# PriUVBio/optiland_Pr

Hardware: AMD Instinct MI355X
Metric: ray-surface intersections/sec at 1M pupil rays, 10-surf double-Gauss (higher is better)
Workload: dtype f64

## Files before the change

### optiland_pr_amd/csrc/ort_fastpath.h

```cpp
#pragma once

#include "ort_core.h"

namespace ort {
namespace fast {

#ifdef ORT_NO_HOSTCONST
#define ORT_TWO_R(s) (2.0 * (s).radius)
#define ORT_ONE_PLUS_K(s) (1.0 + (s).conic)
#define ORT_R_SQ(s) ((s).radius * (s).radius)
#define ORT_U_SQ(u, u_sq) ((u) * (u))
#else
#define ORT_TWO_R(s) ((s).two_r)
#define ORT_ONE_PLUS_K(s) ((s).one_plus_k)
#define ORT_R_SQ(s) ((s).r_sq)
#define ORT_U_SQ(u, u_sq) (u_sq)
#endif

#ifdef ORT_FAST_NOCHECK
#define ORT_CHK(bad, cond) ((void)0)
#else
#define ORT_CHK(bad, cond) ((bad) = (bad) | (cond))
#endif

ORT_INLINE bool is_pos_zero(double v) {
#if defined(__HIP_DEVICE_COMPILE__)
  return __builtin_amdgcn_class(v, 1 << 6);
#else
  return v == 0.0 && !signbit(v);
#endif
}

ORT_INLINE double sqrt(double x, bool& bad) {
#if defined(__HIP_DEVICE_COMPILE__)
  const double y = __builtin_amdgcn_rsq(x);
  double g = x * y;
  double h = y * 0.5;
  const double r = fma(-h, g, 0.5);
  g = fma(g, r, g);
  h = fma(h, r, h);
  double d = fma(-g, g, x);
  g = fma(d, h, g);
  d = fma(-g, g, x);
  g = fma(d, h, g);
  ORT_CHK(bad, !(x >= 0x1p-767));
  return g;
#else
  (void)bad;
  return ::sqrt(x);
#endif
}

ORT_INLINE double sqrt_ge1(double x, bool& bad) {
#if defined(__HIP_DEVICE_COMPILE__)
  const double y = __builtin_amdgcn_rsq(x);
  double g = x * y;
  double h = y * 0.5;
  const double r = fma(-h, g, 0.5);
  g = fma(g, r, g);
  h = fma(h, r, h);
  double d = fma(-g, g, x);
  g = fma(d, h, g);
  d = fma(-g, g, x);
  g = fma(d, h, g);
  (void)bad;
  return g;
#else
  (void)bad;
  return ::sqrt(x);
#endif
}

ORT_INLINE SharedDiv shared_div(double b, bool& bad) {
  SharedDiv d;
  d.b = b;
  d.ok = true;
#if defined(__HIP_DEVICE_COMPILE__)
  double y = __builtin_amdgcn_rcp(b);
  double e = fma(-b, y, 1.0);
  y = fma(y, e, y);
  e = fma(-b, y, 1.0);
  y = fma(y, e, y);
  d.y = y;
  ORT_CHK(bad, !(::fabs(b) <= 0x1p300));
#else
  (void)bad;
  d.y = 0.0;
#endif
  return d;
}

ORT_INLINE SharedDiv shared_div_ge1(double b, bool& bad) {
  SharedDiv d;
  d.b = b;
  d.ok = true;
  (void)bad;
#if defined(__HIP_DEVICE_COMPILE__)
  double y = __builtin_amdgcn_rcp(b);
  double e = fma(-b, y, 1.0);
  y = fma(y, e, y);
  e = fma(-b, y, 1.0);
  y = fma(y, e, y);
  d.y = y;
#else
  (void)bad;
  d.y = 0.0;
#endif
  return d;
}

ORT_INLINE double quot(double a, const SharedDiv& d) {
#if defined(__HIP_DEVICE_COMPILE__)
  const double q0 = a * d.y;
  const double r = fma(-d.b, q0, a);
  return fma(r, d.y, q0);
#else
  return a / d.b;
#endif
}

ORT_INLINE double quot_pos(double a, const SharedDiv& d) {
#if defined(__HIP_DEVICE_COMPILE__)
  const double q0 = a * d.y;
  const double rn = fma(d.b, q0, -a);
  return fma(-rn, d.y, q0);
#else
  return a / d.b;
#endif
}

ORT_INLINE bool num_ok(double a) { return ::fabs(a) >= 0x1p-300; }

ORT_INLINE double sdiv(double a, const SharedDiv& d, bool& bad) {
  ORT_CHK(bad, !num_ok(a));
  return quot(a, d);
}
ORT_INLINE double sdiv0(double a, const SharedDiv& d, bool& bad) {
  ORT_CHK(bad, !(num_ok(a) || is_pos_zero(a)));
  return quot(a, d);
}

ORT_INLINE double div(double a, double b, bool& bad) {
  const SharedDiv d = shared_div(b, bad);
  return sdiv0(a, d, bad);
}

ORT_INLINE Ray generate_ray(const ort_segment& s, double px, double py,
                            const ort_apodization* apod, bool& bad) {
  Ray r;
  double x0, y0;
  if (s.mode == ORT_GEN_INFINITE) {
    x0 = px * s.epd / 2.0 * s.vx + s.x_off;
    y0 = py * s.epd / 2.0 * s.vy + s.y_off;
  } else {
    x0 = s.x_off;
    y0 = s.y_off;
  }
  const double z0 = s.z0;
  double x1, y1;
  if (s.mode == ORT_GEN_TELECENTRIC) {
    x1 = px * s.vx + x0;
    y1 = py * s.vy + y0;
  } else {
    x1 = px * s.epd * s.vx / 2.0;
    y1 = py * s.epd * s.vy / 2.0;
  }
  const double z1 = s.epl;
  const double dx = x1 - x0, dy = y1 - y0, dz = z1 - z0;
  const double mag = sqrt(dx * dx + dy * dy + dz * dz, bad);
  ORT_CHK(bad, (mag < 1e-9));
  const SharedDiv dm = shared_div(mag, bad);
  ORT_CHK(bad, !((num_ok(dx) || dx == 0.0) && (num_ok(dy) || dy == 0.0) &&
                 (num_ok(dz) || dz == 0.0)));
  r.L = quot_pos(dx, dm);
  r.M = quot_pos(dy, dm);
  r.N = quot_pos(dz, dm);
  r.x = x0;
  r.y = y0;
  r.z = z0;
  r.i = apod ? apodize(*apod, px, py) : 1.0;
  r.opd = 0.0;
  r.att = 0.0;
  return r;
}

ORT_INLINE bool state_ok(const Ray& r) {
  constexpr double kMax = 0x1p1000;
  return ::fabs(r.x) < kMax && ::fabs(r.y) < kMax && ::fabs(r.z) < kMax &&
         ::fabs(r.L) < kMax && ::fabs(r.M) < kMax && ::fabs(r.N) < kMax && ::fabs(r.opd) < kMax;
}

ORT_INLINE double distance_plane(const Ray& r, bool& bad) { return div(-r.z, r.N, bad); }

ORT_INLINE double distance_conic(const Ray& r, const ort_surface& s, bool radius_inf,
                                 bool& bad) {
  if (radius_inf) {
    const double Ns = ::fabs(r.N) > 1e-14 ? r.N : 1e-14;
    return div(-r.z, Ns, bad);
  }
  const double R = s.radius, k = s.conic;
  const double N2 = r.N * r.N;
  const double z2 = r.z * r.z;
  double a, b, c;
  if (k == 0.0) {
    a = r.L * r.L + r.M * r.M + N2;
    b = 2.0 * (r.L * r.x + r.M * r.y - r.N * R + r.N * r.z);
    c = 0.0 - ORT_TWO_R(s) * r.z + r.x * r.x + r.y * r.y + z2;
  } else {
    a = k * N2 + r.L * r.L + r.M * r.M + N2;
    b = 2.0 * (k * r.N * r.z + r.L * r.x + r.M * r.y - r.N * R + r.N * r.z);
    c = k * z2 - ORT_TWO_R(s) * r.z + r.x * r.x + r.y * r.y + z2;
  }
  const double d = b * b - 4.0 * a * c;
  const double sd = sqrt(d, bad);
  const SharedDiv a2 = shared_div(2.0 * a, bad);
  const double n1 = -b + sd, n2 = -b - sd;
  ORT_CHK(bad, !(num_ok(n1) && num_ok(n2)));
  const double t1 = quot_pos(n1, a2);
  const double t2 = quot_pos(n2, a2);
  const double z1 = r.z + t1 * r.N;
  const double zz2 = r.z + t2 * r.N;
  return ::fabs(z1) <= ::fabs(zz2) ? t1 : t2;
}

ORT_INLINE void normal_conic_rcp(double x, double y, const ort_surface& s, double& nx,
                                 double& ny, double& nz, bool& bad) {
  const double r2 = x * x + y * y;
  const double a = ORT_ONE_PLUS_K(s) * r2;
  const double q0 = a * s.inv_r2;
  const double q = fma(fma(-ORT_R_SQ(s), q0, a), s.inv_r2, q0);
  const double denom = s.radius * sqrt(1.0 - q, bad);
  const SharedDiv dd = shared_div(denom, bad);
  const double dfdx = sdiv0(x, dd, bad);
  const double dfdy = sdiv0(y, dd, bad);
  const double mag = sqrt_ge1(dfdx * dfdx + dfdy * dfdy + 1.0, bad);
  const SharedDiv dm = shared_div_ge1(mag, bad);
  nx = quot_pos(dfdx, dm);
  ny = quot_pos(dfdy, dm);
  nz = quot(-1.0, dm);
}

ORT_INLINE double align_normal(const Ray& r, double& nx, double& ny, double& nz, bool& bad) {
#ifdef ORT_NO_SIGN_XOR
  return ::ort::align_normal(r, nx, ny, nz);
#endif
  const double dot = r.L * nx + r.M * ny + r.N * nz;
  ORT_CHK(bad, !(::fabs(dot) > 0.0));
  const uint64_t sb = (uint64_t)__double_as_longlong(dot) & 0x8000000000000000ull;
  nx = __longlong_as_double((long long)((uint64_t)__double_as_longlong(nx) ^ sb));
  ny = __longlong_as_double((long long)((uint64_t)__double_as_longlong(ny) ^ sb));
  nz = __longlong_as_double((long long)((uint64_t)__double_as_longlong(nz) ^ sb));
  return ::fabs(dot);
}

ORT_INLINE void refract(Ray& r, double nx, double ny, double nz, double u, double u_sq,
                        bool& bad) {
  const double dot = align_normal(r, nx, ny, nz, bad);
  const double root = sqrt(1.0 - ORT_U_SQ(u, u_sq) * (1.0 - dot * dot), bad);
  const double L0 = r.L, M0 = r.M, N0 = r.N;
  r.L = u * L0 + nx * root - u * nx * dot;
  r.M = u * M0 + ny * root - u * ny * dot;
  r.N = u * N0 + nz * root - u * nz * dot;
}

ORT_INLINE void refract_flat(Ray& r, double u, double u_sq, bool& bad) {
  ORT_CHK(bad, !(::fabs(r.N) > 0.0));
  const double root = sqrt(1.0 - ORT_U_SQ(u, u_sq) * (1.0 - r.N * r.N), bad);
  const double uN = u * r.N;
  const double sroot = ::copysign(root, r.N);
  r.L = u * r.L + 0.0;
  r.M = u * r.M + 0.0;
  r.N = (uN + sroot) - uN;
}

ORT_INLINE double quot_signed(double a, const SharedDiv& d) {
  return d.b > 0.0 ? quot_pos(a, d) : quot(a, d);
}
ORT_INLINE bool num_ok0(double a) { return num_ok(a) || a == 0.0; }

ORT_INLINE SharedDiv shared_div_pos(double b) {
  bool unused = false;
  return shared_div_ge1(b, unused);
}
ORT_INLINE bool lens_range(double R) { return ::fabs(R) <= 0x1p149; }

ORT_INLINE void slope_out(double dfdx, double dfdy, double& nx, double& ny, double& nz,
                          bool& bad) {
#ifdef ORT_SLOPE_MAXCHK
  ORT_CHK(bad, !(::fabs(dfdx) < 7e13 && ::fabs(dfdy) < 7e13));
#else
  ORT_CHK(bad, !(dfdx * dfdx + dfdy * dfdy + 1.0 < 1e28));
#endif
  nx = dfdx;
  ny = dfdy;
  nz = -1.0;
}

ORT_INLINE void unit_normal_from_slope(double dfdx, double dfdy, double& nx, double& ny,
                                       double& nz, bool& bad) {
  const double mag = sqrt_ge1(dfdx * dfdx + dfdy * dfdy + 1.0, bad);
  const SharedDiv dm = shared_div_ge1(mag, bad);
  ORT_CHK(bad, !(num_ok0(dfdx) && num_ok0(dfdy)));
  nx = quot_pos(dfdx, dm);
  ny = quot_pos(dfdy, dm);
  nz = quot(-1.0, dm);
}

template <class PD>
ORT_INLINE double sagnorm_even(double x, double y, const ort_surface& s, PD C,
                               int nc, int mode, double& nx, double& ny, double& nz,
                               bool& bad) {
  const double R = s.radius;
  const double aR = ::fabs(R), sR = R > 0.0 ? 1.0 : -1.0;
  ORT_CHK(bad, !lens_range(R));
  const double r2 = x * x + y * y;
  const double a = ORT_ONE_PLUS_K(s) * r2;
  const SharedDiv rr = shared_div_pos(ORT_R_SQ(s));
  ORT_CHK(bad, !num_ok0(a));
  const double q = sqrt(1.0 - quot_pos(a, rr), bad);
  const SharedDiv dz = shared_div_pos(aR * (1.0 + q));
  ORT_CHK(bad, !num_ok0(r2));
  double P, D;
  ort::even_horner(r2, C, nc, P, D);
  const double z = quot_pos(sR * r2, dz) + r2 * P;
  const SharedDiv dd = shared_div_pos(aR * q);
  ORT_CHK(bad, !(num_ok0(x) && num_ok0(y)));
  double dfdx = quot_pos(sR * x, dd);
  double dfdy = quot_pos(sR * y, dd);
  dfdx = dfdx + x * D;
  dfdy = dfdy + y * D;
  if (mode == kSlope) {
    slope_out(dfdx, dfdy, nx, ny, nz, bad);
    return z;
  }
  const double mag = sqrt_ge1(dfdx * dfdx + dfdy * dfdy + 1.0, bad);
  const SharedDiv dm = shared_div_ge1(mag, bad);
  ORT_CHK(bad, !(num_ok0(dfdx) && num_ok0(dfdy)));
  nx = quot_pos(dfdx, dm);
  ny = quot_pos(dfdy, dm);
  nz = quot(-1.0, dm);
  return z;
}

template <class PD>
ORT_INLINE double sagnorm_odd(double x, double y, const ort_surface& s, PD C,
                              int nc, int mode, double& nx, double& ny, double& nz,
                              bool& bad) {
  const double R = s.radius;
  const double aR = ::fabs(R), sR = R > 0.0 ? 1.0 : -1.0;
  ORT_CHK(bad, !lens_range(R));
  const double r2 = x * x + y * y;
  const double r = sqrt(r2, bad);
  const double a = ORT_ONE_PLUS_K(s) * r2;
  const SharedDiv rr = shared_div_pos(ORT_R_SQ(s));
  ORT_CHK(bad, !num_ok0(a));
  const double q = sqrt(1.0 - quot_pos(a, rr), bad);
  const SharedDiv dz = shared_div_pos(aR * (1.0 + q));
  ORT_CHK(bad, !num_ok0(r2));
  double z = quot_pos(sR * r2, dz);
  double rp = r;
  for (int i = 0; i < nc; ++i) {
    z = z + C[i] * rp;
    rp = rp * r;
  }
  const SharedDiv dd = shared_div_pos(aR * q);
  ORT_CHK(bad, !(num_ok0(x) && num_ok0(y)));
  double dfdx = quot_pos(sR * x, dd);
  double dfdy = quot_pos(sR * y, dd);
  const SharedDiv dr = shared_div(r, bad);
  double rq = quot_pos(1.0, dr);
  for (int i = 0; i < nc; ++i) {
    const double f = (double)(i + 1);
    double xt = f * x * C[i] * rq;
    double yt = f * y * C[i] * rq;
    if (!isfinite(xt)) xt = 0.0;
    if (!isfinite(yt)) yt = 0.0;
    rq = (i == 0) ? 1.0 : (i == 1 ? r : rq * r);
    dfdx = dfdx + xt;
    dfdy = dfdy + yt;
  }
  if (mode == kSlope) {
    slope_out(dfdx, dfdy, nx, ny, nz, bad);
    return z;
  }
  const double mag = sqrt_ge1(dfdx * dfdx + dfdy * dfdy + 1.0, bad);
  const SharedDiv dm = shared_div_ge1(mag, bad);
  ORT_CHK(bad, !(num_ok0(dfdx) && num_ok0(dfdy)));
  nx = quot_pos(dfdx, dm);
  ny = quot_pos(dfdy, dm);
  nz = quot(-1.0, dm);
  return z;
}

ORT_INLINE double newton_step_slope(const Ray& r, double t, double f, double fx, double fy,
                                    bool& bad) {
  const double df = fx * r.L + fy * r.M - r.N;
  const double dfs = ::fabs(df) > 1e-14 ? df : 1e-14;
  const SharedDiv dd = shared_div(dfs, bad);
  ORT_CHK(bad, !num_ok0(f));
  return t - quot_signed(f, dd);
}

ORT_INLINE double newton_step(const Ray& r, double t, double f, double nx, double ny,
                              double nz, bool& bad) {
  const double nzs = ::fabs(nz) > 1e-14 ? nz : 1e-14;
  const SharedDiv dn = shared_div(nzs, bad);
  const double mnx = -nx, mny = -ny;
  ORT_CHK(bad, !(num_ok0(mnx) && num_ok0(mny)));
  const double fx = quot_signed(mnx, dn);
  const double fy = quot_signed(mny, dn);
  const double df = fx * r.L + fy * r.M - r.N;
  const double dfs = ::fabs(df) > 1e-14 ? df : 1e-14;
  const SharedDiv dd = shared_div(dfs, bad);
  ORT_CHK(bad, !num_ok0(f));
  return t - quot_signed(f, dd);
}

}
}
```

### optiland_pr_amd/csrc/ort_kernels.h

```cpp

#pragma once

#include <hip/hip_runtime.h>
#include <stdlib.h>

#include "ort_core.h"
#include "ort_fastpath.h"
#include "ort_interact.h"
#include "ort_material.h"
#include "ort_sweep.h"

namespace ortk {

#ifndef ORT_TEMPORAL_STORE
#define ORT_ST(lhs, v) __builtin_nontemporal_store((v), &(lhs))
#else
#define ORT_ST(lhs, v) ((lhs) = (v))
#endif


constexpr int kBlock = 256;
#ifndef ORT_VERIFY_GRID
#define ORT_VERIFY_GRID 1024
#endif
// ... 531 lines not shown
    bool hn = false;
    double hnx = 0.0, hny = 0.0, hnz = 0.0;
    const bool radius_inf = (s.flags & ORT_SURF_RADIUS_INF) != 0;
    if (!known_geometry(s.geometry)) range_bits |= ORT_STATUS_BAD_GEOMETRY;
    if (s.geometry == ORT_GEOM_PLANE) {
      if constexpr (FAST)
        t = ort::fast::distance_plane(r, bad);
      else
        t = ort::distance_plane(r);
    } else if (s.geometry == ORT_GEOM_STANDARD) {
      if constexpr (FAST)
        t = ort::fast::distance_conic(r, s, radius_inf, bad);
      else
        t = ort::distance_conic(r, s.radius, s.conic, radius_inf);
    } else {
      if constexpr ((FEAT & F_KM) != 0) {
        t = newton_distance<FEAT, FAST>(a, s, si, r, active, group, group_uniform, range_bits,
                                        hn, hnx, hny, hnz, active ? tp : nullptr, sched, bad);
      } else {
        t = __builtin_nan("");
      }
    }
    if constexpr ((FEAT & F_TAPE) != 0) {
      if (active) ORT_ST(tp[6 * a.n_rays], t);
    }
    const double n_pre = o.n_pre, u = o.u, alpha = o.alpha_pre;
    if constexpr ((FEAT & F_IA) != 0) {
      ort::propagate(r, t, alpha);
      if (unnorm) {
        ort::normalize_dir(r);
        unnorm = false;
      }
      ort::add_opd(r, t, n_pre);
      if (s.flags & ORT_SURF_APERTURE) ort::clip_radial(r, s.ap_rmax2, s.ap_rmin2);
      if (s.flags & ORT_SURF_APERTURE_PROG) ort::clip_program(r, cst(a.coef) + s.ap_off, s.ap_len);
      interact<FEAT>(a, s, r, o, lam, wl, unnorm);
    } else if constexpr (FAST) {
      to_intersection(a, s, r, t, alpha, n_pre);
      const bool refl = (s.flags & ORT_SURF_REFLECTIVE) != 0;
      const bool is_plane = s.geometry == ORT_GEOM_PLANE;
      if (!hn && !refl && (is_plane || (radius_inf && s.geometry == ORT_GEOM_STANDARD))) {
        ort::fast::refract_flat(r, u, o.u_sq, bad);
      } else {
        double nx, ny, nz;
        if (hn) {
          nx = hnx; ny = hny; nz = hnz;
        } else if (is_plane) {
          nx = 0.0; ny = 0.0; nz = 1.0;
        } else if (s.flags & ORT_SURF_INV_R2) {
          ort::fast::normal_conic_rcp(r.x, r.y, s, nx, ny, nz, bad);
        } else {
          ort::normal_conic(r.x, r.y, s.radius, s.conic, nx, ny, nz);
        }
        if (refl)
          ort::reflect(r, nx, ny, nz);
        else
          ort::fast::refract(r, nx, ny, nz, u, o.u_sq, bad);
      }
    } else if constexpr ((FEAT & F_KM) != 0) {
      if (hn) {
        to_intersection(a, s, r, t, alpha, n_pre);
        if (s.flags & ORT_SURF_REFLECTIVE)
          ort::reflect(r, hnx, hny, hnz);
        else
          ort::refract(r, hnx, hny, hnz, u);
      } else {
        ort::finish_surface<(FEAT & F_KM)>(r, s, s.radius, s.conic, cst(a.coef), cst(a.zern), kNoSeed, t, n_pre, u,
                                           alpha);
      }
    } else {
      to_intersection<kApProg>(a, s, r, t, alpha, n_pre);
      double nx, ny, nz;
      if (s.geometry == ORT_GEOM_PLANE) {
        nx = 0.0; ny = 0.0; nz = 1.0;
      } else if (s.flags & ORT_SURF_INV_R2) {
        ort::normal_conic_rcp(r.x, r.y, s.radius, s.conic, s.inv_r2, nx, ny, nz);
      } else {
        ort::normal_conic(r.x, r.y, s.radius, s.conic, nx, ny, nz);
      }
      if (s.flags & ORT_SURF_REFLECTIVE)
        ort::reflect(r, nx, ny, nz);
      else
        ort::refract(r, nx, ny, nz, u);
    }
    globalize(a, s, r);
    if constexpr ((FEAT & F_REC) != 0) {
      if ((s.flags & ORT_SURF_RECORD) && active) store_record(a, s, rid, r);
    }
  }
  if (a.final_mat >= 0) {
    ort::propagate(r, a.final_thickness, final_alpha<FEAT>(a, lam, wl));
    if constexpr ((FEAT & F_IA) != 0) {
      if (unnorm) ort::normalize_dir(r);
    }
  }
  return r;
}

template <uint32_t FEAT>
__device__ __forceinline__ void trace_block(const KArgs& a, const int32_t* sched, int64_t vb,
                                            int64_t nb) {
  const int64_t rid =
      a.block_remap ? pair_major_ray(a, vb, nb) : vb * kBlock + threadIdx.x;
  const bool active = rid < a.n_rays;
  const int64_t r_ld = active ? rid : 0;
  bool redo = false;
  if constexpr (kNewtonFast<FEAT>) {
    if (a.newton_mode == ORT_NEWTON_SCHEDULE && !a.exact_only) {
      bool bad = false;
      int fast_bits = 0;
      int64_t fgroup = 0;
      bool fgroup_uniform = true;
      fgroup = r_ld / a.group_len;
      const int64_t g0 = __shfl(fgroup, 0, 64);
      fgroup_uniform = __all(fgroup == g0);
      const ort::Ray rf = trace_ray<FEAT, true>(a, rid, active, fgroup, fgroup_uniform, sched,
                                                fast_bits, bad);
      bad = bad | !ort::fast::state_ok(rf);
#ifdef ORT_FAST_PROBE
      if (bad) {
        ort::Ray rb = rf;
        rb.x = __builtin_nan("");
        if (active) store_ray(a, rid, rb);
        return;
      }
#endif
      if (!bad) {
        if (fast_bits && active && a.status) atomicOr(a.status, fast_bits);
        if (active) store_ray(a, rid, rf);
        return;
      }
      redo = true;
    }
  }

  const int64_t sidx = a.seg ? r_ld / a.seg_len : 0;
  int lam = 0;
  double wl = 0.0;
  ort::Ray r;
  if constexpr (FEAT & F_GEN) {
    const ort_segment sg = a.seg[sidx];
    lam = sg.lambda_idx;
    const int64_t p = a.pupil_per_ray ? r_ld : (r_ld - sidx * a.seg_len);
    r = ort::generate_ray(sg, a.px[p], a.py[p], a.apod);
  } else {
    if (a.seg) lam = a.seg[sidx].lambda_idx;
    if constexpr ((FEAT & F_WRAY) != 0) wl = a.w[r_ld];
    load_ray(a, r_ld, r);
  }
  int64_t group = 0;
  bool group_uniform = true;
  if constexpr ((FEAT & F_KM) != 0) {
    group = r_ld / a.group_len;
    if (redo) {
      group_uniform = false;
    } else {
      const int64_t g0 = __shfl(group, 0, 64);
      group_uniform = __all(group == g0);
    }
  }
  int range_bits = 0;
  bool unnorm = false;
  if constexpr ((FEAT & F_GEN) != 0) {
    if (a.apod && (uint32_t)cst(a.apod)->kind > (uint32_t)ORT_APOD_TUKEY)
      range_bits |= ORT_STATUS_BAD_APODIZATION;
  }

  for (int si = a.start_surface; si < a.n_surf; ++si) {
    const ort_surface s = cst(a.surf)[si];
    const ort_surface_optics o = surface_optics<FEAT>(a, s, lam, si, wl);
    double* tp = nullptr;
    if constexpr ((FEAT & F_TAPE) != 0) {
      tp = a.tape + tape_row0(a.surf, si) * a.n_rays + rid;
      if (active) store_tape_point(a, tp, r);
    }
    localize(a, s, r);
    double t;
    bool hn = false;
    double hnx = 0.0, hny = 0.0, hnz = 0.0;
    if (!known_geometry(s.geometry)) range_bits |= ORT_STATUS_BAD_GEOMETRY;
    if (s.geometry == ORT_GEOM_PLANE) {
      t = ort::distance_plane(r);
    } else if (s.geometry == ORT_GEOM_STANDARD) {
      t = ort::distance_conic(r, s.radius, s.conic, (s.flags & ORT_SURF_RADIUS_INF) != 0);
    } else {
      if constexpr ((FEAT & F_KM) != 0) {
        bool unused = false;
        t = newton_distance<FEAT>(a, s, si, r, active, group, group_uniform, range_bits, hn,
                                  hnx, hny, hnz, active ? tp : nullptr, sched, unused);
      } else {
        t = __builtin_nan("");
      }
    }
    if constexpr ((FEAT & F_TAPE) != 0) {
      if (active) ORT_ST(tp[6 * a.n_rays], t);
    }
    const double n_pre = o.n_pre, u = o.u, alpha = o.alpha_pre;
    if constexpr ((FEAT & F_IA) != 0) {
      ort::propagate(r, t, alpha);
      if (unnorm) {
        ort::normalize_dir(r);
        unnorm = false;
      }
      ort::add_opd(r, t, n_pre);
      if (s.flags & ORT_SURF_APERTURE) ort::clip_radial(r, s.ap_rmax2, s.ap_rmin2);
      if (s.flags & ORT_SURF_APERTURE_PROG) ort::clip_program(r, cst(a.coef) + s.ap_off, s.ap_len);
      interact<FEAT>(a, s, r, o, lam, wl, unnorm);
    } else if constexpr ((FEAT & F_KM) != 0) {
      if (hn) {
        to_intersection(a, s, r, t, alpha, n_pre);
        if (s.flags & ORT_SURF_REFLECTIVE)
          ort::reflect(r, hnx, hny, hnz);
        else
          ort::refract(r, hnx, hny, hnz, u);
      } else {
        ort::finish_surface<(FEAT & F_KM)>(r, s, s.radius, s.conic, cst(a.coef), cst(a.zern), kNoSeed, t, n_pre, u,
                                           alpha);
      }
    } else {
      to_intersection<kApProg>(a, s, r, t, alpha, n_pre);
      double nx, ny, nz;
      if (s.geometry == ORT_GEOM_PLANE) {
        nx = 0.0; ny = 0.0; nz = 1.0;
      } else if (s.flags & ORT_SURF_INV_R2) {
        ort::normal_conic_rcp(r.x, r.y, s.radius, s.conic, s.inv_r2, nx, ny, nz);
      } else {
        ort::normal_conic(r.x, r.y, s.radius, s.conic, nx, ny, nz);
      }
      if (s.flags & ORT_SURF_REFLECTIVE)
        ort::reflect(r, nx, ny, nz);
      else
        ort::refract(r, nx, ny, nz, u);
    }
    globalize(a, s, r);
    if constexpr ((FEAT & F_REC) != 0) {
      if ((s.flags & ORT_SURF_RECORD) && active) store_record(a, s, rid, r);
    }
  }
  if (a.final_mat >= 0) {
    ort::propagate(r, a.final_thickness, final_alpha<FEAT>(a, lam, wl));
    if constexpr ((FEAT & F_IA) != 0) {
      if (unnorm) ort::normalize_dir(r);
    }
  }

  if (range_bits && active && a.status) atomicOr(a.status, range_bits);
  if constexpr ((FEAT & F_RMS) != 0) rms_epilogue(a, r, active, vb);
  if (!active) return;
  store_ray(a, rid, r);
}

template <uint32_t FEAT>
__global__ __launch_bounds__(kBlock) ORT_TRACE_OCC void trace_kernel(const KArgs a) {
  if (a.run_if && *cst(a.run_if) != 1) return;
  const int32_t* sched = a.sched;
  __shared__ int32_t vsched[ORT_VERIFY_MAX_SCHED];
  __shared__ int32_t vcodes[kBlock / 64];
  if constexpr ((FEAT & F_KM) != 0) {
    if (a.vstats) {
      const int64_t ng = (a.n_rays + a.group_len - 1) / a.group_len;
      const int nsch = (int)ng * a.n_surf;
      constexpr int kPre = ORT_VERIFY_MAX_SCHED / kBlock;
      int32_t pre[kPre];
#pragma unroll
      for (int q = 0; q < kPre; ++q) {
        const int k = threadIdx.x + q * kBlock;
        pre[q] = k < nsch ? a.sched[k] : 0;
      }
      const int prev = a.vprev ? *a.vprev : 1;
      if (prev != 1) {
        if (blockIdx.x == 0) {
#pragma unroll
          for (int q = 0; q < kPre; ++q) {
            const int k = threadIdx.x + q * kBlock;
            if (k < nsch) a.sched_out[k] = pre[q];
          }
          if (threadIdx.x == 0) *a.vflag = prev;
        }
        return;
      }
#pragma unroll
      for (int q = 0; q < kPre; ++q) {
        const int k = threadIdx.x + q * kBlock;
        if (k < nsch) vsched[k] = pre[q];
      }
      __syncthreads();
      const int c = newton_decide(a.surf, a.n_surf, ng, a.vstats, a.conv_base, vsched, vcodes);
      if (blockIdx.x == 0) {
        for (int k = threadIdx.x; k < nsch; k += kBlock) a.sched_out[k] = vsched[k];
        if (threadIdx.x == 0) *a.vflag = c;
      }
      if (c != 1) return;
      sched = vsched;
    }
  }
  const int64_t nb = (a.n_rays + kBlock - 1) / kBlock;
  if constexpr ((FEAT & F_STRIDE) != 0) {
    for (int64_t vb = blockIdx.x; vb < nb; vb += gridDim.x) trace_block<FEAT>(a, sched, vb, nb);
  } else {
    trace_block<FEAT>(a, sched, blockIdx.x, nb);
  }
}

template <uint32_t FEAT, bool FAST>
__device__ inline ort::Ray closed_ray_in(const KArgs& a, int64_t r_ld, int& lam, double& wl,
                                         bool& bad) {
  ort::Ray r;
  if constexpr ((FEAT & F_GEN) != 0) {
    const int64_t sidx = a.n_seg == 1 ? 0 : r_ld / a.seg_len;
    const ort_segment sg = a.n_seg == 1 ? cst(a.seg)[0] : a.seg[sidx];
    lam = sg.lambda_idx;
    const int64_t p = a.pupil_per_ray ? r_ld : (r_ld - sidx * a.seg_len);
    if constexpr (FAST)
      r = ort::fast::generate_ray(sg, a.px[p], a.py[p], nullptr, bad);
    else
      r = ort::generate_ray(sg, a.px[p], a.py[p], nullptr);
  } else {
    if (a.seg) lam = a.seg[a.n_seg == 1 ? 0 : r_ld / a.seg_len].lambda_idx;
    if constexpr ((FEAT & F_WRAY) != 0) wl = a.w[r_ld];
    load_ray(a, r_ld, r);
    if constexpr (FAST) bad = bad | !(::fabs(r.L) < __builtin_inf() && ::fabs(r.M) < __builtin_inf());
  }
  return r;
}

template <uint32_t FEAT, bool FAST>
__device__ inline void closed_surfaces(const KArgs& a, ort::Ray& r, int lam, double wl,
                                       int64_t rid, bool active, bool& bad, bool& geom_bad,
                                       double apod = 1.0) {
  for (int si = a.start_surface; si < a.n_surf; ++si) {
    const ort_surface s = cst(a.surf)[si];
    const ort_surface_optics o = surface_optics<FEAT>(a, s, lam, si, wl);
    if constexpr ((FEAT & F_AXIAL) != 0)
      r.z = r.z + -s.cs_t[2];
    else
      localize(a, s, r);
    const bool is_plane = s.geometry == ORT_GEOM_PLANE;
    const bool radius_inf = (s.flags & ORT_SURF_RADIUS_INF) != 0;
    double t;
    if constexpr (FAST) {
      t = is_plane ? ort::fast::distance_plane(r, bad)
                   : ort::fast::distance_conic(r, s, radius_inf, bad);
    } else {
      t = is_plane ? ort::distance_plane(r) : ort::distance_conic(r, s.radius, s.conic, radius_inf);
    }
    if constexpr (FAST) {
      ORT_CHK(bad, s.geometry > ORT_GEOM_STANDARD || s.geometry < ORT_GEOM_PLANE);
    } else if (!is_plane && s.geometry != ORT_GEOM_STANDARD) {
      t = __builtin_nan("");
      geom_bad = true;
    }
#ifndef ORT_NO_ALPHA_FLAGS
    if constexpr ((FEAT & F_WRAY) != 0)
      ort::propagate(r, t, o.alpha_pre);
    else
      ort::propagate_flagged(r, t, o.alpha_pre, s.flags);
#else
    ort::propagate(r, t, o.alpha_pre);
#endif
    ort::add_opd(r, t, o.n_pre);
    if (s.flags & ORT_SURF_APERTURE) ort::clip_radial(r, s.ap_rmax2, s.ap_rmin2);
#ifndef ORT_NO_AP_PROG
    if (s.flags & ORT_SURF_APERTURE_PROG) ort::clip_program(r, cst(a.coef) + s.ap_off, s.ap_len);
#endif
    const bool refl = (s.flags & ORT_SURF_REFLECTIVE) != 0;
#ifndef ORT_NO_FLAT_FAST
    constexpr bool kFlat = FAST;
#else
    constexpr bool kFlat = false;
#endif
    if (kFlat && !refl && (is_plane || radius_inf)) {
      ort::fast::refract_flat(r, o.u, o.u_sq, bad);
    } else {
      double nx, ny, nz;
      if (is_plane) {
        nx = 0.0; ny = 0.0; nz = 1.0;
      } else if (s.flags & ORT_SURF_INV_R2) {
        if constexpr (FAST)
          ort::fast::normal_conic_rcp(r.x, r.y, s, nx, ny, nz, bad);
        else
          ort::normal_conic_rcp(r.x, r.y, s.radius, s.conic, s.inv_r2, nx, ny, nz);
      } else {
        ort::normal_conic(r.x, r.y, s.radius, s.conic, nx, ny, nz);
      }
      if (refl) {
        ort::reflect(r, nx, ny, nz);
      } else {
        if constexpr (FAST)
          ort::fast::refract(r, nx, ny, nz, o.u, o.u_sq, bad);
        else
          ort::refract(r, nx, ny, nz, o.u);
      }
    }
    if constexpr ((FEAT & F_AXIAL) != 0) {
      r.x = r.x + 0.0;
      r.y = r.y + 0.0;
      r.z = r.z + s.cs_t[2];
    } else {
      globalize(a, s, r);
    }
    if constexpr ((FEAT & F_REC) != 0) {
      if ((s.flags & ORT_SURF_RECORD) && active) {
        if constexpr ((FEAT & F_GEN) != 0)
          store_record(a, s, rid, r, a.apod ? &apod : nullptr);
        else
          store_record(a, s, rid, r);
      }
    }
  }
}

template <uint32_t FEAT>
__global__ __launch_bounds__(kClosedBlock) __attribute__((amdgpu_waves_per_eu(8))) void trace_closed_kernel(const KArgs a) {
  int64_t rid;
  bool active;
  if constexpr ((FEAT & F_SPOT) != 0) {
    const int64_t pair = blockIdx.x / a.spot_chunks;
    const int64_t j = (int64_t)(blockIdx.x - pair * a.spot_chunks) * kClosedBlock + threadIdx.x;
    rid = pair * a.seg_len + j;
    active = j < a.seg_len && rid < a.n_rays;
  } else {
    rid = (int64_t)blockIdx.x * kClosedBlock + threadIdx.x;
    active = rid < a.n_rays;
  }
  const int64_t r_ld = active ? rid : 0;
  int lam = 0;
  double wl = 0.0;
  bool bad = false, geom_bad = false;
  double apod_f = 1.0;
  if constexpr ((FEAT & F_GEN) != 0 && (FEAT & F_REC) != 0) {
    if (a.apod) {
      const int64_t sidx = a.n_seg == 1 ? 0 : r_ld / a.seg_len;
      const int64_t p = a.pupil_per_ray ? r_ld : (r_ld - sidx * a.seg_len);
      apod_f = ort::apodize(*cst(a.apod), a.px[p], a.py[p]);
    }
  }
#ifndef ORT_NO_DEFERRED_CHECKS
  ort::Ray r = closed_ray_in<FEAT, true>(a, r_ld, lam, wl, bad);
  closed_surfaces<FEAT, true>(a, r, lam, wl, rid, active, bad, geom_bad, apod_f);
  bad = bad | !ort::fast::state_ok(r);
  if (__builtin_expect(bad, 0)) {
    r = closed_ray_in<FEAT, false>(a, r_ld, lam, wl, bad);
    closed_surfaces<FEAT, false>(a, r, lam, wl, rid, active, bad, geom_bad, apod_f);
  }
#else
  ort::Ray r = closed_ray_in<FEAT, false>(a, r_ld, lam, wl, bad);
  closed_surfaces<FEAT, false>(a, r, lam, wl, rid, active, bad, geom_bad, apod_f);
#endif
  if (a.final_mat >= 0) ort::propagate(r, a.final_thickness, final_alpha<FEAT>(a, lam, wl));
  if (geom_bad && a.status && threadIdx.x == 0) atomicOr(a.status, (int)ORT_STATUS_BAD_GEOMETRY);
  if constexpr ((FEAT & F_GEN) != 0) {
    if (a.apod && a.status && threadIdx.x == 0 &&
        (uint32_t)cst(a.apod)->kind > (uint32_t)ORT_APOD_TUKEY)
      atomicOr(a.status, (int)ORT_STATUS_BAD_APODIZATION);
  }
  double inten = ort::intensity(r);
#ifndef ORT_NO_APOD
  if constexpr ((FEAT & F_GEN) != 0) {
    if (a.apod) {
      const int64_t sidx = a.n_seg == 1 ? 0 : r_ld / a.seg_len;
      const int64_t p = a.pupil_per_ray ? r_ld : (r_ld - sidx * a.seg_len);
      inten = ort::apodize(*cst(a.apod), a.px[p], a.py[p]) * inten;
    }
  }
#endif
  if constexpr ((FEAT & F_SPOT) != 0) spot_epilogue<FEAT>(a, r, inten, active);
  if (!active) return;
  store_ray(a, rid, r, &inten);
}

template <int CTRL, int ROW_MASK>
__device__ inline double dpp_step(double v) {
  const long long b = __double_as_longlong(v);
  const int lo = __builtin_amdgcn_update_dpp(0, (int)(b & 0xffffffffll), CTRL, ROW_MASK, 0xf,
                                             false);
  const int hi = __builtin_amdgcn_update_dpp(0, (int)(b >> 32), CTRL, ROW_MASK, 0xf, false);
  return __longlong_as_double(((long long)hi << 32) | (long long)(unsigned)lo);
}
__device__ inline double wave_sum(double v) {
  if (__builtin_amdgcn_read_exec() == ~0ull) {
    v += dpp_step<0xB1, 0xf>(v);
    v += dpp_step<0x4E, 0xf>(v);
    v += dpp_step<0x141, 0xf>(v);
    v += dpp_step<0x140, 0xf>(v);
    v += dpp_step<0x142, 0xa>(v);
    v += dpp_step<0x143, 0xc>(v);
    const long long b = __double_as_longlong(v);
    const int lo = __builtin_amdgcn_readlane((int)(b & 0xffffffffll), 63);
    const int hi = __builtin_amdgcn_readlane((int)(b >> 32), 63);
    return __longlong_as_double(((long long)hi << 32) | (long long)(unsigned)lo);
  }
  for (int o = 32; o > 0; o >>= 1) v += __shfl_xor(v, o, 64);
  return v;
}

template <int P, uint32_t KM>
__global__ __launch_bounds__(kBlock) void vjp_kernel(const KArgs a, const JArgs j) {
  const int64_t rid = (int64_t)blockIdx.x * kBlock + threadIdx.x;
  const bool active = rid < a.n_rays;
  double acc[P];
  vjp_ray<P, KM>(a, j, rid, active, acc);
  __shared__ double part[kBlock / 64][P];
#pragma unroll
  for (int k = 0; k < P; ++k) {
    const double v = wave_sum(acc[k]);
    if ((threadIdx.x & 63) == 0) part[threadIdx.x >> 6][k] = v;
  }
  __syncthreads();
  if (threadIdx.x < P) {
    double v = 0.0;
#pragma unroll
    for (int w = 0; w < kBlock / 64; ++w) v += part[w][threadIdx.x];
    j.partial[(int64_t)blockIdx.x * P + threadIdx.x] = v;
  }
}

template <int P>
__global__ __launch_bounds__(kBlock) void vjp_reduce_kernel(const JArgs j, int64_t n_block) {
  const int k = blockIdx.x;
  if (j.p0 + k >= j.n_param) return;
  double v = 0.0;
  for (int64_t b = threadIdx.x; b < n_block; b += kBlock) v += j.partial[b * P + k];
  v = wave_sum(v);
  __shared__ double ws[kBlock / 64];
  if ((threadIdx.x & 63) == 0) ws[threadIdx.x >> 6] = v;
  __syncthreads();
  if (threadIdx.x == 0) {
    double s = 0.0;
    for (int w = 0; w < kBlock / 64; ++w) s += ws[w];
    j.grad[j.p0 + k] += s;
  }
}

struct GArgs {
  int32_t surface;
  int32_t mode;
  const double* x;
  const double* y;
  double* sag;
  double* nx;
  double* ny;
  double* nz;
  double* t;
};

template <uint32_t KM>
__global__ __launch_bounds__(kBlock) void geom_kernel(const KArgs a, const GArgs g) {
  const int64_t rid = (int64_t)blockIdx.x * kBlock + threadIdx.x;
  const bool active = rid < a.n_rays;
  const int64_t r_ld = active ? rid : 0;
  const ort_surface s = cst(a.surf)[g.surface];
  bool range_error = false;
  int range_bits = 0;
  if (g.mode == 0) {
    const double x = g.x[r_ld], y = g.y[r_ld];
    double z, nx, ny, nz;
    if (s.geometry == ORT_GEOM_PLANE) {
      z = 0.0;
      nx = 0.0; ny = 0.0; nz = 1.0;
    } else if (s.geometry == ORT_GEOM_STANDARD) {
      z = ort::sag_conic(x * x + y * y, s.radius, s.conic);
      ort::normal_conic(x, y, s.radius, s.conic, nx, ny, nz);
    } else {
      if constexpr (KM != 0) {
        z = ort::newton_sagnorm<KM>(s, s.radius, s.conic, cst(a.coef), cst(a.zern), kNoSeed, x, y, true,
                                    range_error, nx, ny, nz);
      } else {
        z = nx = ny = nz = __builtin_nan("");
      }
    }
    if (active) {
      if (g.sag) g.sag[rid] = z;
      if (g.nx) g.nx[rid] = nx;
      if (g.ny) g.ny[rid] = ny;
      if (g.nz) g.nz[rid] = nz;
    }
  } else {
    ort::Ray r;
    r.x = a.in.x[r_ld];
    r.y = a.in.y[r_ld];
    r.z = a.in.z[r_ld];
    r.L = a.in.L[r_ld];
    r.M = a.in.M[r_ld];
    r.N = a.in.N[r_ld];
    r.i = 1.0;
    r.opd = 0.0;
    r.att = 0.0;
    double t;
    if (s.geometry == ORT_GEOM_PLANE) {
      t = ort::distance_plane(r);
    } else if (s.geometry == ORT_GEOM_STANDARD) {
      t = ort::distance_conic(r, s.radius, s.conic, (s.flags & ORT_SURF_RADIUS_INF) != 0);
    } else {
      if constexpr (KM != 0) {
        bool hn, bad = false;
        double hnx, hny, hnz;
        t = newton_distance<KM>(a, s, g.surface, r, active, 0, true, range_bits, hn, hnx, hny,
                                hnz, nullptr, a.sched, bad);
      } else {
        t = __builtin_nan("");
      }
    }
    if (active && g.t) g.t[rid] = t;
  }
  if (range_error) range_bits |= range_bit(s);
  if (range_bits && active && a.status) atomicOr(a.status, range_bits);
}

typedef void (*KernelFn)(const KArgs);
typedef void (*VjpFn)(const KArgs, const JArgs);
typedef void (*VjpReduceFn)(const JArgs, int64_t);
typedef void (*GeomFn)(const KArgs, const GArgs);

KernelFn select_trace(uint32_t feat);
int closed_block();
KernelFn select_closed(uint32_t feat);
KernelFn select_generate();
KernelFn select_trace_w(uint32_t feat);
KernelFn select_trace_mono(uint32_t feat);
KernelFn select_trace_ia(uint32_t feat);
KernelFn select_trace_tape(uint32_t feat);
void launch_material_nk(const ort_material* mats, const double* coef, int32_t mat,
                        const double* w, int64_t n, double* n_out, double* k_out,
                        hipStream_t stream);
VjpFn select_vjp(int tangents, uint32_t km);
VjpReduceFn select_vjp_reduce(int tangents);
GeomFn select_geom(uint32_t km);
int launch_pupil(const ort_pupil& d, double* px, double* py, hipStream_t stream);

}
```

Measured before the change: 181.6 billion.

## Use wave-ballot fast-path error flags, fold quadratic factor of two, reload kernargs

Templates the fast-path check helpers on the flag type so the per-ray bad flag becomes a wave-wide ballot mask held in scalar registers. Per-surface checks accumulate into a local bool that is ballotted once per surface. The conic intersection uses the half-b form of the quadratic, with an added overflow check on the squared terms. The kernel re-reads kernel arguments through the kernarg pointer after the fast loop, and the no-op axial x/y updates are trimmed to the first surface. The aim is to cut vector-register pressure and ALU work in the hot loop, at the cost of a new exact_only fallback condition and a coarser wave-level bad flag.

```diff
diff --git a/optiland_pr_amd/csrc/ort_fastpath.h b/optiland_pr_amd/csrc/ort_fastpath.h
--- a/optiland_pr_amd/csrc/ort_fastpath.h
+++ b/optiland_pr_amd/csrc/ort_fastpath.h
@@ -19,8 +19,22 @@
 
 #ifdef ORT_FAST_NOCHECK
 #define ORT_CHK(bad, cond) ((void)0)
-#else
-#define ORT_CHK(bad, cond) ((bad) = (bad) | (cond))
+#define ORT_CHK_UNIFORM(bad, cond) ((void)0)
+#else
+#define ORT_CHK(bad, cond) ::ort::fast::chk((bad), (cond))
+#define ORT_CHK_UNIFORM(bad, cond) ::ort::fast::chk_uniform((bad), (cond))
+#endif
+
+struct WaveFlag {
+  uint64_t m;
+};
+ORT_INLINE void chk(bool& bad, bool cond) { bad = bad | cond; }
+ORT_INLINE void chk_uniform(bool& bad, bool cond) { bad = bad | cond; }
+#if defined(__HIPCC__)
+__device__ inline void chk(WaveFlag& bad, bool cond) { bad.m |= __builtin_amdgcn_ballot_w64(cond); }
+__device__ inline void chk_uniform(WaveFlag& bad, bool cond) {
+  if (cond) bad.m = ~0ull;
+}
 #endif
 
 ORT_INLINE bool is_pos_zero(double v) {
@@ -31,7 +45,8 @@
 #endif
 }
 
-ORT_INLINE double sqrt(double x, bool& bad) {
+template <class B>
+ORT_INLINE double sqrt(double x, B& bad) {
 #if defined(__HIP_DEVICE_COMPILE__)
   const double y = __builtin_amdgcn_rsq(x);
   double g = x * y;
@@ -51,7 +66,8 @@
 #endif
 }
 
-ORT_INLINE double sqrt_ge1(double x, bool& bad) {
+template <class B>
+ORT_INLINE double sqrt_ge1(double x, B& bad) {
 #if defined(__HIP_DEVICE_COMPILE__)
   const double y = __builtin_amdgcn_rsq(x);
   double g = x * y;
@@ -71,7 +87,8 @@
 #endif
 }
 
-ORT_INLINE SharedDiv shared_div(double b, bool& bad) {
+template <class B>
+ORT_INLINE SharedDiv shared_div(double b, B& bad) {
   SharedDiv d;
   d.b = b;
   d.ok = true;
@@ -90,7 +107,8 @@
   return d;
 }
 
-ORT_INLINE SharedDiv shared_div_ge1(double b, bool& bad) {
+template <class B>
+ORT_INLINE SharedDiv shared_div_ge1(double b, B& bad) {
   SharedDiv d;
   d.b = b;
   d.ok = true;
@@ -131,22 +149,26 @@
 
 ORT_INLINE bool num_ok(double a) { return ::fabs(a) >= 0x1p-300; }
 
-ORT_INLINE double sdiv(double a, const SharedDiv& d, bool& bad) {
+template <class B>
+ORT_INLINE double sdiv(double a, const SharedDiv& d, B& bad) {
   ORT_CHK(bad, !num_ok(a));
   return quot(a, d);
 }
-ORT_INLINE double sdiv0(double a, const SharedDiv& d, bool& bad) {
+template <class B>
+ORT_INLINE double sdiv0(double a, const SharedDiv& d, B& bad) {
   ORT_CHK(bad, !(num_ok(a) || is_pos_zero(a)));
   return quot(a, d);
 }
 
-ORT_INLINE double div(double a, double b, bool& bad) {
+template <class B>
+ORT_INLINE double div(double a, double b, B& bad) {
   const SharedDiv d = shared_div(b, bad);
   return sdiv0(a, d, bad);
 }
 
+template <class B>
 ORT_INLINE Ray generate_ray(const ort_segment& s, double px, double py,
-                            const ort_apodization* apod, bool& bad) {
+                            const ort_apodization* apod, B& bad) {
   Ray r;
   double x0, y0;
   if (s.mode == ORT_GEN_INFINITE) {
@@ -190,7 +212,8 @@
          ::fabs(r.L) < kMax && ::fabs(r.M) < kMax && ::fabs(r.N) < kMax && ::fabs(r.opd) < kMax;
 }
 
-ORT_INLINE double distance_plane(const Ray& r, bool& bad) { return div(-r.z, r.N, bad); }
+template <class B>
+ORT_INLINE double distance_plane(const Ray& r, B& bad) { return div(-r.z, r.N, bad); }
 
 ORT_INLINE double distance_conic(const Ray& r, const ort_surface& s, bool radius_inf,
                                  bool& bad) {
@@ -223,8 +246,43 @@
   return ::fabs(z1) <= ::fabs(zz2) ? t1 : t2;
 }
 
+template <class B>
+ORT_INLINE double distance_conic_folded(const Ray& r, const ort_surface& s, bool radius_inf,
+                                        B& bad) {
+  if (radius_inf) {
+    const double Ns = ::fabs(r.N) > 1e-14 ? r.N : 1e-14;
+    return div(-r.z, Ns, bad);
+  }
+  const double R = s.radius, k = s.conic;
+  const double N2 = r.N * r.N;
+  const double z2 = r.z * r.z;
+  double a, S, c;
+  if (k == 0.0) {
+    a = r.L * r.L + r.M * r.M + N2;
+    S = r.L * r.x + r.M * r.y - r.N * R + r.N * r.z;
+    c = r.x * r.x - ORT_TWO_R(s) * r.z + r.y * r.y + z2;
+  } else {
+    a = k * N2 + r.L * r.L + r.M * r.M + N2;
+    S = k * r.N * r.z + r.L * r.x + r.M * r.y - r.N * R + r.N * r.z;
+    c = k * z2 - ORT_TWO_R(s) * r.z + r.x * r.x + r.y * r.y + z2;
+  }
+  const double SS = S * S, ac = a * c;
+  ORT_CHK(bad, !(SS < 0x1p1020 && ::fabs(ac) < 0x1p1020));
+  const double d = SS - ac;
+  const double sd = sqrt(d, bad);
+  const SharedDiv a1 = shared_div(a, bad);
+  const double n1 = -S + sd, n2 = -S - sd;
+  ORT_CHK(bad, !(num_ok(n1) && num_ok(n2)));
+  const double t1 = quot_pos(n1, a1);
+  const double t2 = quot_pos(n2, a1);
+  const double z1 = r.z + t1 * r.N;
+  const double zz2 = r.z + t2 * r.N;
+  return ::fabs(z1) <= ::fabs(zz2) ? t1 : t2;
+}
+
+template <class B>
 ORT_INLINE void normal_conic_rcp(double x, double y, const ort_surface& s, double& nx,
-                                 double& ny, double& nz, bool& bad) {
+                                 double& ny, double& nz, B& bad) {
   const double r2 = x * x + y * y;
   const double a = ORT_ONE_PLUS_K(s) * r2;
   const double q0 = a * s.inv_r2;
@@ -240,7 +298,8 @@
   nz = quot(-1.0, dm);
 }
 
-ORT_INLINE double align_normal(const Ray& r, double& nx, double& ny, double& nz, bool& bad) {
+template <class B>
+ORT_INLINE double align_normal(const Ray& r, double& nx, double& ny, double& nz, B& bad) {
 #ifdef ORT_NO_SIGN_XOR
   return ::ort::align_normal(r, nx, ny, nz);
 #endif
@@ -253,8 +312,9 @@
   return ::fabs(dot);
 }
 
+template <class B>
 ORT_INLINE void refract(Ray& r, double nx, double ny, double nz, double u, double u_sq,
-                        bool& bad) {
+                        B& bad) {
   const double dot = align_normal(r, nx, ny, nz, bad);
   const double root = sqrt(1.0 - ORT_U_SQ(u, u_sq) * (1.0 - dot * dot), bad);
   const double L0 = r.L, M0 = r.M, N0 = r.N;
@@ -263,7 +323,8 @@
   r.N = u * N0 + nz * root - u * nz * dot;
 }
 
-ORT_INLINE void refract_flat(Ray& r, double u, double u_sq, bool& bad) {
+template <class B>
+ORT_INLINE void refract_flat(Ray& r, double u, double u_sq, B& bad) {
   ORT_CHK(bad, !(::fabs(r.N) > 0.0));
   const double root = sqrt(1.0 - ORT_U_SQ(u, u_sq) * (1.0 - r.N * r.N), bad);
   const double uN = u * r.N;
diff --git a/optiland_pr_amd/csrc/ort_kernels.h b/optiland_pr_amd/csrc/ort_kernels.h
--- a/optiland_pr_amd/csrc/ort_kernels.h
+++ b/optiland_pr_amd/csrc/ort_kernels.h
@@ -857,9 +857,9 @@
   }
 }
 
-template <uint32_t FEAT, bool FAST>
+template <uint32_t FEAT, bool FAST, class B>
 __device__ inline ort::Ray closed_ray_in(const KArgs& a, int64_t r_ld, int& lam, double& wl,
-                                         bool& bad) {
+                                         B& bad) {
   ort::Ray r;
   if constexpr ((FEAT & F_GEN) != 0) {
     const int64_t sidx = a.n_seg == 1 ? 0 : r_ld / a.seg_len;
@@ -874,14 +874,14 @@
     if (a.seg) lam = a.seg[a.n_seg == 1 ? 0 : r_ld / a.seg_len].lambda_idx;
     if constexpr ((FEAT & F_WRAY) != 0) wl = a.w[r_ld];
     load_ray(a, r_ld, r);
-    if constexpr (FAST) bad = bad | !(::fabs(r.L) < __builtin_inf() && ::fabs(r.M) < __builtin_inf());
+    if constexpr (FAST) ORT_CHK(bad, !(::fabs(r.L) < __builtin_inf() && ::fabs(r.M) < __builtin_inf()));
   }
   return r;
 }
 
-template <uint32_t FEAT, bool FAST>
+template <uint32_t FEAT, bool FAST, class B>
 __device__ inline void closed_surfaces(const KArgs& a, ort::Ray& r, int lam, double wl,
-                                       int64_t rid, bool active, bool& bad, bool& geom_bad,
+                                       int64_t rid, bool active, B& bad, bool& geom_bad,
                                        double apod = 1.0) {
   for (int si = a.start_surface; si < a.n_surf; ++si) {
     const ort_surface s = cst(a.surf)[si];
@@ -892,15 +892,16 @@
       localize(a, s, r);
     const bool is_plane = s.geometry == ORT_GEOM_PLANE;
     const bool radius_inf = (s.flags & ORT_SURF_RADIUS_INF) != 0;
+    bool sbad = false;
     double t;
     if constexpr (FAST) {
-      t = is_plane ? ort::fast::distance_plane(r, bad)
-                   : ort::fast::distance_conic(r, s, radius_inf, bad);
+      t = is_plane ? ort::fast::distance_plane(r, sbad)
+                   : ort::fast::distance_conic_folded(r, s, radius_inf, sbad);
     } else {
       t = is_plane ? ort::distance_plane(r) : ort::distance_conic(r, s.radius, s.conic, radius_inf);
     }
     if constexpr (FAST) {
-      ORT_CHK(bad, s.geometry > ORT_GEOM_STANDARD || s.geometry < ORT_GEOM_PLANE);
+      ORT_CHK_UNIFORM(bad, s.geometry > ORT_GEOM_STANDARD || s.geometry < ORT_GEOM_PLANE);
     } else if (!is_plane && s.geometry != ORT_GEOM_STANDARD) {
       t = __builtin_nan("");
       geom_bad = true;
@@ -925,14 +926,14 @@
     constexpr bool kFlat = false;
 #endif
     if (kFlat && !refl && (is_plane || radius_inf)) {
-      ort::fast::refract_flat(r, o.u, o.u_sq, bad);
+      ort::fast::refract_flat(r, o.u, o.u_sq, sbad);
     } else {
       double nx, ny, nz;
       if (is_plane) {
         nx = 0.0; ny = 0.0; nz = 1.0;
       } else if (s.flags & ORT_SURF_INV_R2) {
         if constexpr (FAST)
-          ort::fast::normal_conic_rcp(r.x, r.y, s, nx, ny, nz, bad);
+          ort::fast::normal_conic_rcp(r.x, r.y, s, nx, ny, nz, sbad);
         else
           ort::normal_conic_rcp(r.x, r.y, s.radius, s.conic, s.inv_r2, nx, ny, nz);
       } else {
@@ -942,18 +943,22 @@
         ort::reflect(r, nx, ny, nz);
       } else {
         if constexpr (FAST)
-          ort::fast::refract(r, nx, ny, nz, o.u, o.u_sq, bad);
+          ort::fast::refract(r, nx, ny, nz, o.u, o.u_sq, sbad);
         else
           ort::refract(r, nx, ny, nz, o.u);
       }
     }
     if constexpr ((FEAT & F_AXIAL) != 0) {
-      r.x = r.x + 0.0;
-      r.y = r.y + 0.0;
+      if (!FAST || si == a.start_surface) {
+        if constexpr (FAST) asm volatile("");
+        r.x = r.x + 0.0;
+        r.y = r.y + 0.0;
+      }
       r.z = r.z + s.cs_t[2];
     } else {
       globalize(a, s, r);
     }
+    if constexpr (FAST) ORT_CHK(bad, sbad);
     if constexpr ((FEAT & F_REC) != 0) {
       if ((s.flags & ORT_SURF_RECORD) && active) {
         if constexpr ((FEAT & F_GEN) != 0)
@@ -965,8 +970,15 @@
   }
 }
 
+__device__ inline const KArgs& kernarg_again() {
+  auto p = (const __attribute__((address_space(4))) KArgs*)__builtin_amdgcn_kernarg_segment_ptr();
+  asm volatile("" : "+s"(p));
+  return (const KArgs&)*p;
+}
+
 template <uint32_t FEAT>
-__global__ __launch_bounds__(kClosedBlock) __attribute__((amdgpu_waves_per_eu(8))) void trace_closed_kernel(const KArgs a) {
+__global__ __launch_bounds__(kClosedBlock) __attribute__((amdgpu_waves_per_eu(8))) void trace_closed_kernel(const KArgs a0) {
+  const KArgs& a = a0;
   int64_t rid;
   bool active;
   if constexpr ((FEAT & F_SPOT) != 0) {
@@ -991,37 +1003,41 @@
     }
   }
 #ifndef ORT_NO_DEFERRED_CHECKS
-  ort::Ray r = closed_ray_in<FEAT, true>(a, r_ld, lam, wl, bad);
-  closed_surfaces<FEAT, true>(a, r, lam, wl, rid, active, bad, geom_bad, apod_f);
-  bad = bad | !ort::fast::state_ok(r);
+  ort::fast::WaveFlag fbad{0};
+  ort::Ray r = closed_ray_in<FEAT, true>(a, r_ld, lam, wl, fbad);
+  closed_surfaces<FEAT, true>(a, r, lam, wl, rid, active, fbad, geom_bad, apod_f);
+  const KArgs& b = kernarg_again();
+  bad = ((fbad.m >> (threadIdx.x & 63)) & 1) != 0 || !ort::fast::state_ok(r) ||
+        b.exact_only != 0;
   if (__builtin_expect(bad, 0)) {
-    r = closed_ray_in<FEAT, false>(a, r_ld, lam, wl, bad);
-    closed_surfaces<FEAT, false>(a, r, lam, wl, rid, active, bad, geom_bad, apod_f);
+    r = closed_ray_in<FEAT, false>(b, r_ld, lam, wl, bad);
+    closed_surfaces<FEAT, false>(b, r, lam, wl, rid, active, bad, geom_bad, apod_f);
   }
 #else
-  ort::Ray r = closed_ray_in<FEAT, false>(a, r_ld, lam, wl, bad);
-  closed_surfaces<FEAT, false>(a, r, lam, wl, rid, active, bad, geom_bad, apod_f);
-#endif
-  if (a.final_mat >= 0) ort::propagate(r, a.final_thickness, final_alpha<FEAT>(a, lam, wl));
-  if (geom_bad && a.status && threadIdx.x == 0) atomicOr(a.status, (int)ORT_STATUS_BAD_GEOMETRY);
+  const KArgs& b = a;
+  ort::Ray r = closed_ray_in<FEAT, false>(b, r_ld, lam, wl, bad);
+  closed_surfaces<FEAT, false>(b, r, lam, wl, rid, active, bad, geom_bad, apod_f);
+#endif
+  if (b.final_mat >= 0) ort::propagate(r, b.final_thickness, final_alpha<FEAT>(b, lam, wl));
+  if (geom_bad && b.status && threadIdx.x == 0) atomicOr(b.status, (int)ORT_STATUS_BAD_GEOMETRY);
   if constexpr ((FEAT & F_GEN) != 0) {
-    if (a.apod && a.status && threadIdx.x == 0 &&
-        (uint32_t)cst(a.apod)->kind > (uint32_t)ORT_APOD_TUKEY)
-      atomicOr(a.status, (int)ORT_STATUS_BAD_APODIZATION);
+    if (b.apod && b.status && threadIdx.x == 0 &&
+        (uint32_t)cst(b.apod)->kind > (uint32_t)ORT_APOD_TUKEY)
+      atomicOr(b.status, (int)ORT_STATUS_BAD_APODIZATION);
   }
   double inten = ort::intensity(r);
 #ifndef ORT_NO_APOD
   if constexpr ((FEAT & F_GEN) != 0) {
-    if (a.apod) {
-      const int64_t sidx = a.n_seg == 1 ? 0 : r_ld / a.seg_len;
-      const int64_t p = a.pupil_per_ray ? r_ld : (r_ld - sidx * a.seg_len);
-      inten = ort::apodize(*cst(a.apod), a.px[p], a.py[p]) * inten;
-    }
-  }
-#endif
-  if constexpr ((FEAT & F_SPOT) != 0) spot_epilogue<FEAT>(a, r, inten, active);
+    if (b.apod) {
+      const int64_t sidx = b.n_seg == 1 ? 0 : r_ld / b.seg_len;
+      const int64_t p = b.pupil_per_ray ? r_ld : (r_ld - sidx * b.seg_len);
+      inten = ort::apodize(*cst(b.apod), b.px[p], b.py[p]) * inten;
+    }
+  }
+#endif
+  if constexpr ((FEAT & F_SPOT) != 0) spot_epilogue<FEAT>(b, r, inten, active);
   if (!active) return;
-  store_ray(a, rid, r, &inten);
+  store_ray(b, rid, r, &inten);
 }
 
 template <int CTRL, int ROW_MASK>
```

Result: faster. 189.6 billion, median of 6 (+4.5%).
